# DanbiAubrey/Hypergraph_diffusion_for_recommendation

Hardware: AMD Instinct MI355X
Metric: hypergraph-conv fwd+bwd M-edges/sec at emb_dim=64; % HBM roofline (higher is better)
Workload: dtype f32

## Files before the change

hypergraph_diffusion_for_recommendation_amd/_native.py:

```python
from __future__ import annotations

import ctypes
import os
import threading

_HERE = os.path.dirname(os.path.abspath(__file__))
LIB_PATH = os.environ.get("HGD_LIB_PATH", os.path.join(_HERE, "_lib", "libhgd.so"))

c_void_p = ctypes.c_void_p
c_i64 = ctypes.c_int64
c_i32 = ctypes.c_int32
c_f32 = ctypes.c_float
c_f64 = ctypes.c_double
c_size = ctypes.c_size_t

HGD_OK = 0
EPI_NONE, EPI_LEAKY_RELU, EPI_RELU = 0, 1, 2
DT_F32, DT_BF16 = 0, 1
PACKED_IDX_BITS, PACKED_MAX_DICT = 22, 1024
ORDER_NONE, ORDER_MIN_COLUMN, ORDER_GREEDY = 0, 1, 2
ORDER_COL_CAP = 1024
_STATUS_NAMES = {0: "HGD_OK", 1: "HGD_ERR_INVALID_ARG", 2: "HGD_ERR_HIP",
                 3: "HGD_ERR_UNSUPPORTED", 4: "HGD_ERR_WORKSPACE"}

# ... 226 lines not shown
                                    c_i64, c_void_p, c_i32, c_i64, c_void_p, c_i32, c_i64, c_i32,
                                    c_i32, c_f32, c_i32, c_void_p, c_size, c_void_p]),
    "hgd_spmm_blocks_for_dt": (c_i32, [c_i64, c_i32, c_i32]),
    "hgd_spmm_row_order_for": (c_i32, [c_i64, c_i64, c_i64, c_i32]),
    "hgd_spmm_row_order_workspace_size": (c_size, [c_i64]),
    "hgd_spmm_row_order": (c_i32, [c_void_p, c_void_p, c_i64, c_i64, c_void_p, c_void_p,
                                   c_void_p, c_void_p, c_void_p, c_size, c_void_p]),
    "hgd_spmm_ordered": (c_i32, [c_void_p, c_void_p, c_void_p, c_void_p, c_i64, c_i64, c_i64,
                                 c_i64, c_void_p, c_i64, c_void_p, c_i64, c_i32, c_i32, c_f32,
                                 ctypes.POINTER(SplitPlan), c_void_p, c_size, c_void_p,
                                 c_void_p]),
    "hgd_spmm_block_order_for": (c_i32, [c_i64, c_i64, c_i64, c_i32, c_i32]),
    "hgd_spmm_col_blocks_ordered_workspace_size": (c_size, [c_i64, c_i32]),
    "hgd_spmm_col_blocks_ordered": (c_i32, [c_void_p, c_void_p, c_i64, c_i64, c_i32, c_void_p,
                                            c_void_p, c_void_p, c_void_p, c_void_p, c_size,
                                            c_void_p]),
    "hgd_spmm_blocked_ordered": (c_i32, [c_void_p, c_void_p, c_void_p, c_void_p, c_void_p, c_i64,
                                         c_i64, c_void_p, c_i64, c_void_p, c_i64, c_i32, c_i32,
                                         c_f32, c_i32, c_void_p]),
    "hgd_row_order_greedy": (c_i32, [c_void_p, c_void_p, c_i64, c_i64, c_i64, c_i32, c_i32, c_i32,
                                     c_i32, c_i32, c_void_p]),
    "hgd_col_block_order_greedy": (c_i32, [c_void_p, c_void_p, c_i64, c_i64, c_i32, c_i64, c_i32,
                                           c_i32, c_i32, c_i32, c_i32, c_void_p]),
    "hgd_spmm_row_order_from_workspace_size": (c_size, [c_i64]),
    "hgd_spmm_row_order_from": (c_i32, [c_void_p, c_void_p, c_void_p, c_i64, c_i64, c_void_p,
                                        c_void_p, c_void_p, c_void_p, c_size, c_void_p]),
    "hgd_spmm_col_blocks_ordered_from_workspace_size": (c_size, [c_i64, c_i32]),
    "hgd_spmm_col_blocks_ordered_from": (c_i32, [c_void_p, c_void_p, c_void_p, c_i64, c_i64, c_i32,
                                                 c_void_p, c_void_p, c_void_p, c_void_p, c_size,
                                                 c_void_p]),
    "hgd_spmm_order_geometry": (c_i32, [c_i32, c_i32, ctypes.POINTER(c_i32),
                                        ctypes.POINTER(c_i64)]),
    "hgd_spmm_row_order_kind_for": (c_i32, [c_i64, c_i64, c_i64, c_i32, c_i32]),
    "hgd_spmm_packed_for": (c_i32, [c_i64, c_i32, c_i64, c_i32]),
    "hgd_spmm_packed_fits": (c_i32, [c_i64, c_i32, c_i64, c_i32]),
    "hgd_spmm_pack_entries": (c_i32, [c_void_p, c_void_p, c_void_p, c_i64, c_i64, c_i64, c_i32,
                                      c_i32, c_i32, c_void_p, c_void_p]),
    "hgd_spmm_blocked_packed": (c_i32, [c_void_p, c_void_p, c_void_p, c_i32, c_i32, c_void_p,
                                        c_void_p, c_i64, c_i64, c_void_p, c_i64, c_void_p, c_i64,
                                        c_i32, c_i32, c_f32, c_i32, c_void_p]),
    "hgd_spmm_blocked_split_workspace_size": (c_size, [ctypes.POINTER(SplitPlan), c_i32, c_i32]),
    "hgd_spmm_blocked_split": (c_i32, [c_void_p, c_void_p, c_void_p, c_void_p, c_i64, c_i64,
                                       c_i64, c_i64, c_void_p, c_i64, c_void_p, c_i64, c_i32,
                                       c_i32, c_f32, c_i32, ctypes.POINTER(SplitPlan), c_void_p,
                                       c_size, c_void_p]),
    "hgd_spmm_blocks_split_for": (c_i32, [c_i64, c_i32, c_i64, c_i64, c_i32]),
# ... 381 lines not shown
```

hypergraph_diffusion_for_recommendation_amd/csrc/row_order_greedy.cpp:

```cpp
#include <algorithm>
#include <atomic>
#include <cstdarg>
#include <cstdint>
#include <cstdio>
#include <cstdlib>
#include <exception>
#include <new>
#include <thread>
#include <vector>

#include "../../include/hgd.h"

namespace hgd {

extern thread_local char g_last_error[512];

namespace {

hgd_status greedy_fail(hgd_status st, const char* fmt, ...) {
  va_list ap;
  va_start(ap, fmt);
  vsnprintf(g_last_error, sizeof(g_last_error), fmt, ap);
  va_end(ap);
  return st;
}

constexpr int kPickScan = 8;

struct Pieces {
  const int64_t* pb;
// ... 142 lines not shown
      const long v = std::strtol(e, nullptr, 10);
      if (v >= 1) t = v;
    }
  }
  t = std::min<int64_t>(t, n_tasks);
  return static_cast<int>(std::max<int64_t>(t, 1));
}

struct Task {
  Pieces p;
  const int32_t* rows;
  int64_t m;
  int32_t* out;
};

hgd_status run_tasks(const char* fn, const std::vector<Task>& tasks, int64_t window,
                     int64_t col_cap, int32_t threads) {
  std::atomic<size_t> next{0};
  std::atomic<int> bad_column{0}, no_memory{0};
  auto work = [&]() noexcept {
    for (size_t i = next.fetch_add(1); i < tasks.size(); i = next.fetch_add(1)) {
      const Task& t = tasks[i];
      try {
        if (!greedy_chunk(t.p, t.rows, t.m, window, col_cap, t.out)) bad_column.store(1);
      } catch (const std::exception&) {
        no_memory.store(1);
      }
    }
  };
  const int n = pick_threads(threads, static_cast<int64_t>(tasks.size()));
  std::vector<std::thread> th;
  try {
    th.reserve(static_cast<size_t>(n));
    for (int i = 1; i < n; ++i) th.emplace_back(work);
  } catch (const std::exception&) {
  }
  work();
  for (auto& t : th) t.join();
  if (bad_column.load())
    return greedy_fail(HGD_ERR_INVALID_ARG, "%s: a column outside [0, n_cols)", fn);
  if (no_memory.load()) return greedy_fail(HGD_ERR_WORKSPACE, "%s: out of host memory", fn);
  return HGD_OK;
}

void add_tasks(const Pieces& p, const int32_t* ne, int64_t m, int64_t R, int64_t X, int64_t C,
               int32_t* seq, std::vector<Task>& tasks, std::vector<int64_t>& part_off) {
  const int64_t n_wg = (m + R - 1) / R;
  part_off.assign(static_cast<size_t>(X) + 1, 0);
  for (int64_t x = 0; x < X; ++x) {
    const int64_t wgs = n_wg / X + (x < n_wg % X ? 1 : 0);
    int64_t size = wgs * R;
    if (n_wg > 0 && (n_wg - 1) % X == x) size -= n_wg * R - m;
    part_off[static_cast<size_t>(x) + 1] = part_off[static_cast<size_t>(x)] + size;
    for (int64_t c = 0; c < C; ++c) {
      const int64_t b = part_off[static_cast<size_t>(x)] + size * c / C;
      const int64_t e = part_off[static_cast<size_t>(x)] + size * (c + 1) / C;
      if (e > b) tasks.push_back(Task{p, ne + b, e - b, seq + b});
    }
  }
}

void place_parts(const int32_t* seq, const std::vector<int64_t>& part_off, int64_t R, int64_t X,
                 int32_t* order) {
  for (int64_t x = 0; x < X; ++x) {
    const int64_t off = part_off[static_cast<size_t>(x)];
    const int64_t size = part_off[static_cast<size_t>(x) + 1] - off;
    for (int64_t t = 0; t < size; ++t) order[(X * (t / R) + x) * R + t % R] = seq[off + t];
  }
}

hgd_status check_common(const char* fn, const int64_t* rowptr, const int32_t* col, int64_t n_rows,
                        int64_t n_cols, int64_t window, int32_t col_cap, int32_t rows_per_wg,
                        int32_t n_xcd, int32_t chunks_per_xcd, int32_t threads, const void* out) {
  if (n_rows < 0 || n_cols < 0) return greedy_fail(HGD_ERR_INVALID_ARG, "%s: negative sizes", fn);
  if (n_rows >= 0x7fffffffLL || n_cols >= 0x7fffffffLL)
    return greedy_fail(HGD_ERR_INVALID_ARG, "%s: n_rows / n_cols >= 2^31 - 1", fn);
  if (window < 1 || window > 0x7fffffffLL)
    return greedy_fail(HGD_ERR_INVALID_ARG, "%s: window must be 1..2^31-1 (got %lld)", fn,
                       static_cast<long long>(window));
  if (col_cap < 1) return greedy_fail(HGD_ERR_INVALID_ARG, "%s: col_cap must be >= 1", fn);
  if (rows_per_wg < 1 || n_xcd < 1 || chunks_per_xcd < 1)
    return greedy_fail(HGD_ERR_INVALID_ARG,
                       "%s: rows_per_wg, n_xcd and chunks_per_xcd must be >= 1", fn);
  if (threads < 0) return greedy_fail(HGD_ERR_INVALID_ARG, "%s: threads must be >= 0", fn);
  if (n_rows > 0 && (!rowptr || !out))
    return greedy_fail(HGD_ERR_INVALID_ARG, "%s: null rowptr / output", fn);
  if (n_rows > 0) {
    if (rowptr[0] < 0) return greedy_fail(HGD_ERR_INVALID_ARG, "%s: rowptr[0] < 0", fn);
    for (int64_t r = 0; r < n_rows; ++r)
      if (rowptr[r + 1] < rowptr[r])
        return greedy_fail(HGD_ERR_INVALID_ARG, "%s: rowptr descends at row %lld", fn,
                           static_cast<long long>(r));
    if (rowptr[n_rows] > rowptr[0] && !col)
      return greedy_fail(HGD_ERR_INVALID_ARG, "%s: null col", fn);
  }
  return HGD_OK;
}

}
}

extern "C" hgd_status hgd_row_order_greedy(const int64_t* rowptr, const int32_t* col,
                                           int64_t n_rows, int64_t n_cols, int64_t window,
                                           int32_t col_cap, int32_t rows_per_wg, int32_t n_xcd,
                                           int32_t chunks_per_xcd, int32_t threads,
                                           int32_t* order_out) {
  using namespace hgd;
  constexpr const char* fn = "hgd_row_order_greedy";
  g_last_error[0] = '\0';
  hgd_status s = check_common(fn, rowptr, col, n_rows, n_cols, window, col_cap, rows_per_wg, n_xcd,
                              chunks_per_xcd, threads, order_out);
  if (s != HGD_OK || n_rows == 0) return s;
  try {
    std::vector<int32_t> ne, seq;
    int64_t n_empty = 0;
    for (int64_t r = 0; r < n_rows; ++r)
      if (rowptr[r + 1] > rowptr[r]) ne.push_back(static_cast<int32_t>(r));
    const int64_t m = static_cast<int64_t>(ne.size());
    for (int64_t r = 0; r < n_rows; ++r)
      if (rowptr[r + 1] == rowptr[r]) order_out[m + n_empty++] = static_cast<int32_t>(r);
    seq.resize(ne.size());
    const Pieces p{rowptr, rowptr + 1, 1, col, 0, n_cols};
    std::vector<Task> tasks;
    std::vector<int64_t> part_off;
    add_tasks(p, ne.data(), m, rows_per_wg, n_xcd, chunks_per_xcd, seq.data(), tasks, part_off);
    s = run_tasks(fn, tasks, window, col_cap, threads);
    if (s != HGD_OK) return s;
    place_parts(seq.data(), part_off, rows_per_wg, n_xcd, order_out);
  } catch (const std::exception&) {
    return greedy_fail(HGD_ERR_WORKSPACE, "%s: out of host memory", fn);
  }
  return HGD_OK;
}

extern "C" hgd_status hgd_col_block_order_greedy(const int64_t* rowptr, const int32_t* col,
                                                 int64_t n_rows, int64_t n_cols, int32_t n_blocks,
                                                 int64_t window, int32_t col_cap,
                                                 int32_t rows_per_wg, int32_t n_xcd,
                                                 int32_t chunks_per_xcd, int32_t threads,
                                                 int32_t* blk_order_out) {
  using namespace hgd;
  constexpr const char* fn = "hgd_col_block_order_greedy";
  g_last_error[0] = '\0';
  if (n_blocks < 1 || n_blocks > 64)
    return greedy_fail(HGD_ERR_INVALID_ARG, "%s: blocks must be 1..64", fn);
  hgd_status s = check_common(fn, rowptr, col, n_rows, n_cols, window, col_cap, rows_per_wg, n_xcd,
                              chunks_per_xcd, threads, blk_order_out);
  if (s != HGD_OK || n_rows == 0) return s;
  try {
    const int64_t P = n_blocks;
    std::vector<int64_t> cut(static_cast<size_t>(n_rows) * static_cast<size_t>(P + 1));
    for (int64_t r = 0; r < n_rows; ++r) {
      int64_t* c = cut.data() + r * (P + 1);
      int64_t k = 0, prev = -1;
      c[0] = rowptr[r];
      for (int64_t j = rowptr[r]; j < rowptr[r + 1]; ++j) {
        const int64_t v = col[j];
        if (v < prev || v < 0 || v >= n_cols)
          return greedy_fail(HGD_ERR_INVALID_ARG,
                             "%s: row %lld's columns do not ascend inside [0, n_cols)", fn,
                             static_cast<long long>(r));
        prev = v;
        while (k + 1 < P && v >= n_cols * (k + 1) / P) c[++k] = j;
      }
      while (k < P) c[++k] = rowptr[r + 1];
    }
    std::vector<int32_t> ne(static_cast<size_t>(n_rows) * static_cast<size_t>(P));
    std::vector<int32_t> seq(ne.size());
    std::vector<int64_t> m(static_cast<size_t>(P), 0);
    std::vector<std::vector<int64_t>> part_off(static_cast<size_t>(P));
    std::vector<Task> tasks;
    for (int64_t k = 0; k < P; ++k) {
      int32_t* nek = ne.data() + k * n_rows;
      int32_t* outk = blk_order_out + k * n_rows;
      int64_t n_empty = 0, mk = 0;
      for (int64_t r = 0; r < n_rows; ++r)
        if (cut[r * (P + 1) + k + 1] > cut[r * (P + 1) + k]) nek[mk++] = static_cast<int32_t>(r);
      for (int64_t r = 0; r < n_rows; ++r)
        if (cut[r * (P + 1) + k + 1] == cut[r * (P + 1) + k])
          outk[mk + n_empty++] = static_cast<int32_t>(r);
      m[static_cast<size_t>(k)] = mk;
      const Pieces p{cut.data() + k, cut.data() + k + 1, P + 1, col, n_cols * k / P,
                     n_cols * (k + 1) / P};
      add_tasks(p, nek, mk, rows_per_wg, n_xcd, chunks_per_xcd, seq.data() + k * n_rows, tasks,
                part_off[static_cast<size_t>(k)]);
    }
    s = run_tasks(fn, tasks, window, col_cap, threads);
    if (s != HGD_OK) return s;
    for (int64_t k = 0; k < P; ++k)
      place_parts(seq.data() + k * n_rows, part_off[static_cast<size_t>(k)], rows_per_wg, n_xcd,
                  blk_order_out + k * n_rows);
  } catch (const std::exception&) {
    return greedy_fail(HGD_ERR_WORKSPACE, "%s: out of host memory", fn);
  }
  return HGD_OK;
}
```

hypergraph_diffusion_for_recommendation_amd/incidence.py:

```python
from __future__ import annotations

import copy
import ctypes
import os
import weakref
from typing import Dict, Optional, Tuple

import torch

from . import _native as nat
from . import profiling

DEFAULT_SPLIT_THRESHOLD = 2048
DEFAULT_SPLIT_CHUNK = 512
SPLIT_THRESHOLD_MIN = 128
SPLIT_NNZ_PER_THRESHOLD = 8192
SEGMENTED_MAX_AVG_DEGREE = 32
TARGET_GROUPS = 16384
ORDER_XCDS = 8
ORDER_CHUNKS_PER_XCD = 1


def auto_split(n_rows: int, nnz: int) -> Tuple[int, int]:
    if n_rows >= TARGET_GROUPS or nnz == 0:
        t = SPLIT_THRESHOLD_MIN
        while 2 * t <= nnz // SPLIT_NNZ_PER_THRESHOLD and t < DEFAULT_SPLIT_THRESHOLD:
            t *= 2
        return t, min(t // 2, DEFAULT_SPLIT_CHUNK)
    want = max(1, nnz // TARGET_GROUPS)
    chunk = 32
    while chunk < want and chunk < DEFAULT_SPLIT_CHUNK:
        chunk *= 2
    return 2 * chunk, chunk


def _ws(nbytes: int, device) -> torch.Tensor:
    return torch.empty(max(int(nbytes), 1), dtype=torch.uint8, device=device)


def _stream(device) -> int:
    return nat.stream_handle(device)


# ... 164 lines not shown
                ws = _ws(lib.hgd_split_plan_workspace_size(n), dev)
                for k, (n_heavy, n_chunks) in enumerate(counts.tolist()):
                    if n_heavy == 0:
                        continue
                    heavy_rows = torch.empty(n_heavy, dtype=torch.int32, device=dev)
                    heavy_cptr = torch.empty(n_heavy + 1, dtype=torch.int64, device=dev)
                    chunk_heavy = torch.empty(n_chunks, dtype=torch.int32, device=dev)
                    nat.check(lib.hgd_split_plan_build(
                        start.data_ptr() + 8 * k * n, n, thr, chunk, heavy_rows.data_ptr(),
                        heavy_cptr.data_ptr(), chunk_heavy.data_ptr(), n_heavy, n_chunks,
                        ws.data_ptr(), ws.numel(), st), "hgd_split_plan_build")
                    arrays.append((heavy_rows, heavy_cptr, chunk_heavy))
                    p = plans[k]
                    p.threshold, p.chunk = thr, chunk
                    p.n_heavy, p.n_chunks = n_heavy, n_chunks
                    p.heavy_rows = heavy_rows.data_ptr()
                    p.heavy_cptr = heavy_cptr.data_ptr()
                    p.chunk_heavy = chunk_heavy.data_ptr()
            got = self._col_block_plans[n_blocks] = (plans, arrays)
        return got[0]

    def _greedy_order(self, n_blocks: int, geom: tuple) -> torch.Tensor:
        window, rows_per_wg, n_xcd, chunks = geom
        rowptr, col = self.rowptr.cpu().contiguous(), self.col.cpu().contiguous()
        lib = nat.load()
        out = torch.empty(max(1, n_blocks) * self.n_rows, dtype=torch.int32)
        cp = col.data_ptr() if self.nnz else None
        if n_blocks:
            nat.check(lib.hgd_col_block_order_greedy(
                rowptr.data_ptr(), cp, self.n_rows, self.n_cols, n_blocks, window,
                nat.ORDER_COL_CAP, rows_per_wg, n_xcd, chunks, 0, out.data_ptr()),
                "hgd_col_block_order_greedy")
        else:
            nat.check(lib.hgd_row_order_greedy(
                rowptr.data_ptr(), cp, self.n_rows, self.n_cols, window, nat.ORDER_COL_CAP,
                rows_per_wg, n_xcd, chunks, 0, out.data_ptr()), "hgd_row_order_greedy")
        return out.to(self.device)

    def col_blocks_ordered(self, n_blocks: int, kind: int = nat.ORDER_MIN_COLUMN,
                           geom: Optional[tuple] = None) -> Tuple[torch.Tensor, ...]:
        if kind == nat.ORDER_GREEDY:
            return self._col_blocks_greedy(n_blocks, _need_geom(geom))
        got = self._col_blocks_ord.get(n_blocks)
        if got is None:
            if not self.cols_ascending:
                raise RuntimeError(
                    "col_blocks_ordered: the rows' columns are not known to be ascending")
            dev = self.device
            lib = nat.load()
            start = torch.empty(n_blocks * self.n_rows + 1, dtype=torch.int64, device=dev)
            bcol = torch.empty(self.nnz, dtype=torch.int32, device=dev)
            perm = torch.empty(self.nnz, dtype=torch.int32, device=dev)
            out_row = torch.empty(n_blocks * self.n_rows, dtype=torch.int32, device=dev)
            if self.n_rows:
                ws = _ws(lib.hgd_spmm_col_blocks_ordered_workspace_size(self.n_rows, n_blocks),
                         dev)
                nat.check(lib.hgd_spmm_col_blocks_ordered(
                    self.rowptr.data_ptr(), self.col.data_ptr() if self.nnz else None,
                    self.n_rows, self.n_cols, n_blocks, start.data_ptr(),
# ... 897 lines not shown
```

include/hgd.h:

```cpp
#ifndef HGD_H
#define HGD_H

#include <stddef.h>
#include <stdint.h>

#ifdef __cplusplus
extern "C" {
#endif

typedef enum hgd_status {
  HGD_OK = 0,
  HGD_ERR_INVALID_ARG = 1,
  HGD_ERR_HIP = 2,
  HGD_ERR_UNSUPPORTED = 3,
  HGD_ERR_WORKSPACE = 4
} hgd_status;

typedef enum hgd_epilogue {
  HGD_EPI_NONE = 0,
  HGD_EPI_LEAKY_RELU = 1,
  HGD_EPI_RELU = 2
} hgd_epilogue;

typedef enum hgd_tune_key {
// ... 109 lines not shown
                                       int64_t n_cols, int32_t n_blocks, int64_t* blk_start,
                                       int32_t* blk_col, int32_t* blk_perm, int32_t* blk_out_row,
                                       void* workspace, size_t workspace_bytes, void* stream);
hgd_status hgd_spmm_blocked_ordered(const int64_t* blk_start, const int32_t* blk_col,
                                    const float* blk_val, const float* blk_row_scale,
                                    const int32_t* blk_out_row, int64_t n_rows,
                                    int64_t n_src_rows, const float* X, int64_t ldx, float* Y,
                                    int64_t ldy, int32_t d, int32_t epilogue, float slope,
                                    int32_t n_blocks, void* stream);

#define HGD_ORDER_NONE 0
#define HGD_ORDER_MIN_COLUMN 1
#define HGD_ORDER_GREEDY 2
#define HGD_ORDER_COL_CAP 1024
hgd_status hgd_row_order_greedy(const int64_t* rowptr, const int32_t* col, int64_t n_rows,
                                int64_t n_cols, int64_t window, int32_t col_cap,
                                int32_t rows_per_wg, int32_t n_xcd, int32_t chunks_per_xcd,
                                int32_t threads, int32_t* order_out);
hgd_status hgd_col_block_order_greedy(const int64_t* rowptr, const int32_t* col, int64_t n_rows,
                                      int64_t n_cols, int32_t n_blocks, int64_t window,
                                      int32_t col_cap, int32_t rows_per_wg, int32_t n_xcd,
                                      int32_t chunks_per_xcd, int32_t threads,
                                      int32_t* blk_order_out);
size_t hgd_spmm_row_order_from_workspace_size(int64_t n_rows);
hgd_status hgd_spmm_row_order_from(const int32_t* order, const int64_t* rowptr, const int32_t* col,
                                   int64_t n_rows, int64_t n_cols, int64_t* rowptr_o,
                                   int32_t* col_o, int32_t* perm, void* workspace,
                                   size_t workspace_bytes, void* stream);
size_t hgd_spmm_col_blocks_ordered_from_workspace_size(int64_t n_rows, int32_t n_blocks);
hgd_status hgd_spmm_col_blocks_ordered_from(const int32_t* blk_order, const int64_t* rowptr,
                                            const int32_t* col, int64_t n_rows, int64_t n_cols,
                                            int32_t n_blocks, int64_t* blk_start, int32_t* blk_col,
                                            int32_t* blk_perm, void* workspace,
                                            size_t workspace_bytes, void* stream);
int32_t hgd_spmm_order_geometry(int32_t d, int32_t blocked, int32_t* rows_per_wg, int64_t* window);
int32_t hgd_spmm_row_order_kind_for(int64_t n_rows, int64_t n_src_rows, int64_t nnz, int32_t d,
                                    int32_t n_blocks);

#define HGD_SPMM_PACKED_MAX_DICT 1024
#define HGD_SPMM_PACKED_IDX_BITS 22
int32_t hgd_spmm_packed_fits(int64_t n_src_rows, int32_t n_blocks, int64_t n_dict,
                             int32_t idx_bits);
int32_t hgd_spmm_packed_for(int64_t n_src_rows, int32_t n_blocks, int64_t n_dict,
                            int32_t idx_bits);
hgd_status hgd_spmm_pack_entries(const int64_t* blk_start, const int32_t* blk_col,
                                 const int32_t* src_code, int64_t n_rows, int64_t n_src_rows,
// ... 608 lines not shown
```

Before: 7393.

## Add pooled multi-XCD greedy row ordering with a parallel team walk

Result: faster. 7641 (median of 6 runs) (+3.4%).

```diff
diff --git a/hypergraph_diffusion_for_recommendation_amd/_native.py b/hypergraph_diffusion_for_recommendation_amd/_native.py
--- a/hypergraph_diffusion_for_recommendation_amd/_native.py
+++ b/hypergraph_diffusion_for_recommendation_amd/_native.py
@@ -272,6 +272,10 @@
                                      c_i32, c_i32, c_void_p]),
     "hgd_col_block_order_greedy": (c_i32, [c_void_p, c_void_p, c_i64, c_i64, c_i32, c_i64, c_i32,
                                            c_i32, c_i32, c_i32, c_i32, c_void_p]),
+    "hgd_row_order_greedy_pooled": (c_i32, [c_void_p, c_void_p, c_i64, c_i64, c_i64, c_i32, c_i32,
+                                            c_i32, c_i32, c_i32, c_void_p]),
+    "hgd_col_block_order_greedy_pooled": (c_i32, [c_void_p, c_void_p, c_i64, c_i64, c_i32, c_i64,
+                                                  c_i32, c_i32, c_i32, c_i32, c_i32, c_void_p]),
     "hgd_spmm_row_order_from_workspace_size": (c_size, [c_i64]),
     "hgd_spmm_row_order_from": (c_i32, [c_void_p, c_void_p, c_void_p, c_i64, c_i64, c_void_p,
                                         c_void_p, c_void_p, c_void_p, c_size, c_void_p]),
diff --git a/hypergraph_diffusion_for_recommendation_amd/csrc/row_order_greedy.cpp b/hypergraph_diffusion_for_recommendation_amd/csrc/row_order_greedy.cpp
--- a/hypergraph_diffusion_for_recommendation_amd/csrc/row_order_greedy.cpp
+++ b/hypergraph_diffusion_for_recommendation_amd/csrc/row_order_greedy.cpp
@@ -5,7 +5,10 @@
 #include <cstdio>
 #include <cstdlib>
 #include <exception>
+#include <limits>
+#include <memory>
 #include <new>
+#include <stdexcept>
 #include <thread>
 #include <vector>
 
@@ -194,51 +197,600 @@
     for (size_t i = next.fetch_add(1); i < tasks.size(); i = next.fetch_add(1)) {
       const Task& t = tasks[i];
       try {
-        if (!greedy_chunk(t.p, t.rows, t.m, window, col_cap, t.out)) bad_column.store(1);
+          if (!greedy_chunk(t.p, t.rows, t.m, window, col_cap, t.out)) bad_column.store(1);
+        } catch (const std::exception&) {
+          no_memory.store(1);
+        }
+      }
+    };
+    const int n = pick_threads(threads, static_cast<int64_t>(tasks.size()));
+    std::vector<std::thread> th;
+    try {
+      th.reserve(static_cast<size_t>(n));
+      for (int i = 1; i < n; ++i) th.emplace_back(work);
+    } catch (const std::exception&) {
+    }
+    work();
+    for (auto& t : th) t.join();
+    if (bad_column.load())
+      return greedy_fail(HGD_ERR_INVALID_ARG, "%s: a column outside [0, n_cols)", fn);
+    if (no_memory.load()) return greedy_fail(HGD_ERR_WORKSPACE, "%s: out of host memory", fn);
+    return HGD_OK;
+  }
+
+  void add_tasks(const Pieces& p, const int32_t* ne, int64_t m, int64_t R, int64_t X, int64_t C,
+                 int32_t* seq, std::vector<Task>& tasks, std::vector<int64_t>& part_off) {
+    const int64_t n_wg = (m + R - 1) / R;
+    part_off.assign(static_cast<size_t>(X) + 1, 0);
+    for (int64_t x = 0; x < X; ++x) {
+      const int64_t wgs = n_wg / X + (x < n_wg % X ? 1 : 0);
+      int64_t size = wgs * R;
+      if (n_wg > 0 && (n_wg - 1) % X == x) size -= n_wg * R - m;
+      part_off[static_cast<size_t>(x) + 1] = part_off[static_cast<size_t>(x)] + size;
+      for (int64_t c = 0; c < C; ++c) {
+        const int64_t b = part_off[static_cast<size_t>(x)] + size * c / C;
+        const int64_t e = part_off[static_cast<size_t>(x)] + size * (c + 1) / C;
+        if (e > b) tasks.push_back(Task{p, ne + b, e - b, seq + b});
+      }
+    }
+  }
+
+  void place_parts(const int32_t* seq, const std::vector<int64_t>& part_off, int64_t R, int64_t X,
+                   int32_t* order) {
+    for (int64_t x = 0; x < X; ++x) {
+      const int64_t off = part_off[static_cast<size_t>(x)];
+      const int64_t size = part_off[static_cast<size_t>(x) + 1] - off;
+      for (int64_t t = 0; t < size; ++t) order[(X * (t / R) + x) * R + t % R] = seq[off + t];
+    }
+  }
+
+  constexpr int kMaxOwners = 16;
+  constexpr int64_t kMaxRowsPerRound = 8, kRoundShare = 128;
+
+  class TeamBarrier {
+   public:
+    explicit TeamBarrier(int n) : n_(n) {}
+    void wait() {
+      if (n_ == 1) return;
+      const int g = gen_.load(std::memory_order_acquire);
+      if (count_.fetch_add(1, std::memory_order_acq_rel) + 1 == n_) {
+        count_.store(0, std::memory_order_relaxed);
+        gen_.store(g + 1, std::memory_order_release);
+        return;
+      }
+      for (int spin = 0; gen_.load(std::memory_order_acquire) == g; ++spin)
+        if (spin >= 512) std::this_thread::yield();
+    }
+
+   private:
+    const int n_;
+    std::atomic<int> count_{0}, gen_{0};
+  };
+
+  struct Pool {
+    Pieces p;
+    const int32_t* rows;
+    int64_t m;
+    int32_t* seq;
+    std::vector<int64_t> size, off;
+    int64_t nnz, max_len;
+    int K;
+  };
+
+  struct alignas(64) Proposal {
+    int32_t cnt, n;
+    int32_t row[kPickScan];
+    uint16_t len[kPickScan];
+  };
+  static_assert(sizeof(Proposal) == 64, "a proposal is a cache line");
+
+  constexpr int kRecentCols = 32;
+  constexpr int kStackLook = 64;
+
+  template <class Cnt>
+  struct Owner {
+    static constexpr Cnt kPlaced = std::numeric_limits<Cnt>::max();
+    int64_t lo = 0, n = 0;
+    std::vector<uint32_t> tptr;
+    std::vector<int32_t> tl, len;
+    std::vector<Cnt> cnt;
+    std::vector<std::vector<int32_t>> stack;
+    std::vector<int32_t> top;
+    std::vector<uint8_t> mark;
+    int64_t live = 0, gone = 0;
+  };
+
+  template <class Cnt>
+  struct PoolState {
+    std::vector<Owner<Cnt>> owners;
+    std::vector<int32_t> key, by_min, coldeg;
+    std::vector<uint8_t> placed;
+    std::vector<int32_t> in_fifo;
+    std::vector<std::vector<int32_t>> fifo;
+    std::vector<int64_t> fifo_at, fifo_n;
+    std::vector<std::vector<uint32_t>> events;
+    std::vector<int32_t> recent;
+    std::vector<int64_t> recent_n;
+    std::vector<Proposal> prop;
+    std::atomic<int> bad_column{0}, no_memory{0};
+    std::atomic<int> fail_apply{0}, fail_fifo{0};
+  };
+
+  struct Team {
+    explicit Team(int n) : size(n), barrier(n) {}
+    int size;
+    TeamBarrier barrier;
+    void* state = nullptr;
+  };
+
+  template <class Cnt>
+  bool build_owner(const Pool& pl, int G, Owner<Cnt>& o, int32_t* key) {
+    const Pieces& p = pl.p;
+    const int64_t nc = p.c_hi - p.c_lo;
+    o.tptr.assign(static_cast<size_t>(nc) + 1, 0);
+    o.len.resize(static_cast<size_t>(o.n));
+    uint64_t total = 0;
+    for (int64_t i = 0; i < o.n; ++i) {
+      const int32_t r = pl.rows[o.lo + i];
+      const int64_t b = p.begin(r), e = p.end(r);
+      int64_t lo = nc;
+      for (int64_t j = b; j < e; ++j) {
+        const int64_t c = static_cast<int64_t>(p.col[j]) - p.c_lo;
+        if (c < 0 || c >= nc) return false;
+        ++o.tptr[static_cast<size_t>(c) + 1];
+        lo = std::min(lo, c);
+      }
+      key[o.lo + i] = static_cast<int32_t>(lo);
+      o.len[static_cast<size_t>(i)] = static_cast<int32_t>(e - b);
+      total += static_cast<uint64_t>(e - b);
+    }
+    if (total > 0xffffffffull) throw std::length_error("an owner's lists");
+    for (size_t c = 0; c < static_cast<size_t>(nc); ++c) o.tptr[c + 1] += o.tptr[c];
+    o.tl.resize(static_cast<size_t>(total));
+    {
+      std::vector<uint32_t> fill(o.tptr.begin(), o.tptr.end() - 1);
+      for (int64_t i = 0; i < o.n; ++i) {
+        const int32_t r = pl.rows[o.lo + i];
+        for (int64_t j = p.begin(r), e = p.end(r); j < e; ++j)
+          o.tl[fill[static_cast<size_t>(p.col[j] - p.c_lo)]++] = static_cast<int32_t>(i);
+      }
+    }
+    o.cnt.assign(static_cast<size_t>(G) * static_cast<size_t>(o.n), 0);
+    o.stack.assign(static_cast<size_t>(G) * static_cast<size_t>(pl.max_len + 1), {});
+    o.top.assign(static_cast<size_t>(G), 0);
+    o.mark.assign(static_cast<size_t>(o.n), 0);
+    o.live = o.n;
+    return true;
+  }
+
+  template <class Cnt>
+  void pack_lists(Owner<Cnt>& o) {
+    const size_t nc = o.tptr.size() - 1;
+    uint32_t w = 0, j = 0;
+    for (size_t c = 0; c < nc; ++c) {
+      const uint32_t e = o.tptr[c + 1];
+      o.tptr[c] = w;
+      for (; j < e; ++j)
+        if (o.cnt[static_cast<size_t>(o.tl[j])] != Owner<Cnt>::kPlaced) o.tl[w++] = o.tl[j];
+    }
+    o.tptr[nc] = w;
+    o.live -= o.gone;
+    o.gone = 0;
+  }
+
+  inline void offer(Proposal& out, int32_t len32, int32_t row) {
+    const uint16_t len = static_cast<uint16_t>(std::min<int32_t>(len32, 0xffff));
+    for (int i = 0; i < out.n; ++i)
+      if (out.row[i] == row) return;
+    int at = out.n++;
+    for (; at > 0 && (out.len[at - 1] > len || (out.len[at - 1] == len && out.row[at - 1] > row));
+         --at) {
+      out.len[at] = out.len[at - 1];
+      out.row[at] = out.row[at - 1];
+    }
+    out.len[at] = len;
+    out.row[at] = row;
+  }
+
+  template <class Cnt>
+  void sweep(Owner<Cnt>& o, const Cnt* cn, std::vector<int32_t>& st, int32_t b) {
+    size_t w = st.size();
+    for (size_t i = st.size(); i-- > 0;) {
+      const int32_t t = st[i];
+      if (static_cast<int32_t>(cn[t]) != b || o.mark[static_cast<size_t>(t)]) continue;
+      o.mark[static_cast<size_t>(t)] = 1;
+      st[--w] = t;
+    }
+    for (size_t i = w; i < st.size(); ++i) o.mark[static_cast<size_t>(st[i])] = 0;
+    st.erase(st.begin(), st.begin() + static_cast<std::ptrdiff_t>(w));
+  }
+
+  template <class Cnt>
+  void propose(Owner<Cnt>& o, int g, int64_t max_len, const int32_t* recent, int64_t recent_n,
+               Proposal& out) {
+    const Cnt* const cn = o.cnt.data() + static_cast<size_t>(g) * static_cast<size_t>(o.n);
+    std::vector<int32_t>* const stk =
+        o.stack.data() + static_cast<size_t>(g) * static_cast<size_t>(max_len + 1);
+    int32_t top = o.top[static_cast<size_t>(g)];
+    for (; top >= 2; --top) {
+      std::vector<int32_t>& st = stk[top];
+      while (!st.empty() && static_cast<int32_t>(cn[st.back()]) != top) st.pop_back();
+      if (!st.empty()) break;
+    }
+    o.top[static_cast<size_t>(g)] = top;
+    out.n = 0;
+    if (top >= 2) {
+      out.cnt = top;
+      const std::vector<int32_t>& st = stk[top];
+      const size_t stop = st.size() > kStackLook ? st.size() - kStackLook : 0;
+      for (size_t i = st.size(); i-- > stop && out.n < kPickScan;) {
+        const int32_t t = st[i];
+        if (static_cast<int32_t>(cn[t]) == top)
+          offer(out, o.len[static_cast<size_t>(t)], static_cast<int32_t>(o.lo + t));
+      }
+      return;
+    }
+    out.cnt = 1;
+    const int64_t back = std::min<int64_t>(recent_n, kRecentCols);
+    for (int64_t q = 1; q <= back && out.n < kPickScan; ++q) {
+      const size_t c = static_cast<size_t>(recent[(recent_n - q) % kRecentCols]);
+      for (uint32_t j = o.tptr[c], e = o.tptr[c + 1]; j < e && out.n < kPickScan; ++j) {
+        const int32_t t = o.tl[j];
+        if (cn[t] != Owner<Cnt>::kPlaced && cn[t] >= 1)
+          offer(out, o.len[static_cast<size_t>(t)], static_cast<int32_t>(o.lo + t));
+      }
+    }
+  }
+
+  template <class Cnt>
+  void apply_round(Owner<Cnt>& o, int G, int64_t max_len,
+                   const std::vector<std::vector<uint32_t>>& events, std::vector<uint64_t>& evs,
+                   std::vector<uint64_t>& moves) {
+    constexpr size_t kAhead = 8, kMoveAhead = 16;
+    evs.clear();
+    moves.clear();
+    for (int g = 0; g < G; ++g)
+      for (const uint32_t ev : events[static_cast<size_t>(g)])
+        evs.push_back(static_cast<uint64_t>(ev) << 16 | static_cast<uint64_t>(g));
+    const uint32_t* const tptr = o.tptr.data();
+    const int32_t* const tl = o.tl.data();
+    const size_t ne = evs.size();
+    for (size_t i = 0; i < std::min(ne, 2 * kAhead); ++i) __builtin_prefetch(tptr + (evs[i] >> 17));
+    for (size_t i = 0; i < std::min(ne, kAhead); ++i) __builtin_prefetch(tl + tptr[evs[i] >> 17]);
+    for (size_t i = 0; i < ne; ++i) {
+      if (i + 2 * kAhead < ne) __builtin_prefetch(tptr + (evs[i + 2 * kAhead] >> 17));
+      if (i + kAhead < ne) __builtin_prefetch(tl + tptr[evs[i + kAhead] >> 17]);
+      const size_t c = static_cast<size_t>(evs[i] >> 17);
+      const uint64_t low = (evs[i] & 0xffffu) << 1 | (evs[i] >> 16 & 1u);
+      for (uint32_t j = tptr[c], e = tptr[c + 1]; j < e; ++j)
+        moves.push_back(static_cast<uint64_t>(static_cast<uint32_t>(tl[j])) << 32 | low);
+    }
+    Cnt* const cnt = o.cnt.data();
+    const size_t n = static_cast<size_t>(o.n), nm = moves.size();
+    const size_t sweep_at = 2 * n + 256;
+    auto at = [&](uint64_t mv) { return cnt + (mv >> 1 & 0xffffu) * n + (mv >> 32); };
+    for (size_t i = 0; i < std::min(nm, kMoveAhead); ++i) __builtin_prefetch(at(moves[i]), 1);
+    for (size_t i = 0; i < nm; ++i) {
+      if (i + kMoveAhead < nm) __builtin_prefetch(at(moves[i + kMoveAhead]), 1);
+      const uint64_t mv = moves[i];
+      Cnt* const cn = at(mv);
+      const Cnt b = *cn;
+      if (b == Owner<Cnt>::kPlaced) continue;
+      int32_t to;
+      if (mv & 1u) {
+        *cn = static_cast<Cnt>(b + 1);
+        if (b < 1) continue;
+        to = static_cast<int32_t>(b) + 1;
+      } else {
+        if (b < 1) continue;
+        *cn = static_cast<Cnt>(b - 1);
+        if (b < 3) continue;
+        to = static_cast<int32_t>(b) - 1;
+      }
+      const size_t g = mv >> 1 & 0xffffu;
+      std::vector<int32_t>& st =
+          o.stack[g * static_cast<size_t>(max_len + 1) + static_cast<size_t>(to)];
+      if (st.size() >= sweep_at) sweep(o, cnt + g * n, st, to);
+      st.push_back(static_cast<int32_t>(mv >> 32));
+      if ((mv & 1u) && to > o.top[g]) o.top[g] = to;
+    }
+  }
+
+  template <class Cnt>
+  int walk_pool(Team& team, int me, const Pool& pl, int64_t window, int64_t col_cap) {
+    const int G = static_cast<int>(pl.size.size());
+    const int K = pl.K, T = team.size;
+    const Pieces& p = pl.p;
+    const int64_t nc = p.c_hi - p.c_lo, m = pl.m;
+    const int k_lo = K * me / T, k_hi = K * (me + 1) / T;
+    window = std::min<int64_t>(window, std::max<int64_t>(1, pl.nnz));
+
+    if (me == 0) {
+      PoolState<Cnt>* made = nullptr;
+      try {
+        made = new PoolState<Cnt>();
+        made->owners.resize(static_cast<size_t>(K));
+        for (int k = 0; k < K; ++k) {
+          made->owners[static_cast<size_t>(k)].lo = m * k / K;
+          made->owners[static_cast<size_t>(k)].n = m * (k + 1) / K - m * k / K;
+        }
+        made->key.resize(static_cast<size_t>(m));
+        made->by_min.resize(static_cast<size_t>(m));
+        made->coldeg.assign(static_cast<size_t>(nc), 0);
+        made->placed.assign(static_cast<size_t>(m), 0);
+        made->in_fifo.assign(static_cast<size_t>(G) * static_cast<size_t>(nc), 0);
+        made->fifo.resize(static_cast<size_t>(G));
+        for (int g = 0; g < G; ++g)
+          made->fifo[static_cast<size_t>(g)].resize(
+              static_cast<size_t>(std::min(window, pl.size[static_cast<size_t>(g)] * pl.max_len)));
+        made->fifo_at.assign(static_cast<size_t>(G), 0);
+        made->fifo_n.assign(static_cast<size_t>(G), 0);
+        made->events.resize(static_cast<size_t>(G));
+        made->recent.assign(static_cast<size_t>(G) * kRecentCols, 0);
+        made->recent_n.assign(static_cast<size_t>(G), 0);
+        made->prop.resize(static_cast<size_t>(K) * static_cast<size_t>(G));
       } catch (const std::exception&) {
-        no_memory.store(1);
-      }
-    }
-  };
-  const int n = pick_threads(threads, static_cast<int64_t>(tasks.size()));
+        delete made;
+        made = nullptr;
+      }
+      team.state = made;
+    }
+    team.barrier.wait();
+    PoolState<Cnt>* const st = static_cast<PoolState<Cnt>*>(team.state);
+    if (!st) {
+      team.barrier.wait();
+      return 2;
+    }
+
+    for (int k = k_lo; k < k_hi; ++k) {
+      try {
+        if (!build_owner(pl, G, st->owners[static_cast<size_t>(k)], st->key.data()))
+          st->bad_column.store(1);
+      } catch (const std::exception&) {
+        st->no_memory.store(1);
+      }
+    }
+    team.barrier.wait();
+    int bad = st->bad_column.load() ? 1 : st->no_memory.load() ? 2 : 0;
+    if (!bad) {
+      for (int64_t c = nc * me / T, e = nc * (me + 1) / T; c < e; ++c) {
+        int64_t deg = 0;
+        for (int k = 0; k < K; ++k) {
+          const Owner<Cnt>& o = st->owners[static_cast<size_t>(k)];
+          deg += o.tptr[static_cast<size_t>(c) + 1] - o.tptr[static_cast<size_t>(c)];
+        }
+        st->coldeg[static_cast<size_t>(c)] =
+            static_cast<int32_t>(std::min<int64_t>(deg, 0x7fffffff));
+      }
+      if (me == T - 1) {
+      try {
+          std::vector<int64_t> at(static_cast<size_t>(nc) + 2, 0);
+          const int32_t* const key = st->key.data();
+          for (int64_t i = 0; i < m; ++i) ++at[static_cast<size_t>(key[i]) + 1];
+          for (size_t c = 0; c <= static_cast<size_t>(nc); ++c) at[c + 1] += at[c];
+          for (int64_t i = 0; i < m; ++i)
+            st->by_min[static_cast<size_t>(at[static_cast<size_t>(key[i])]++)] =
+                static_cast<int32_t>(i);
+      } catch (const std::exception&) {
+        st->no_memory.store(1);
+      }
+    }
+    team.barrier.wait();
+    bad = st->no_memory.load() ? 2 : 0;
+  }
+
+  if (!bad) {
+    const int64_t B = std::clamp<int64_t>(window * m / (kRoundShare * pl.nnz), 1, kMaxRowsPerRound);
+    int64_t longest = 0;
+    for (int g = 0; g < G; ++g) longest = std::max(longest, pl.size[static_cast<size_t>(g)]);
+    int64_t fall = 0;
+    std::vector<int32_t> pick;
+    std::vector<uint64_t> evs, moves;
+    try {
+      pick.resize(static_cast<size_t>(G) * static_cast<size_t>(B));
+    } catch (const std::exception&) {
+      st->fail_apply.store(1);
+    }
+    const uint8_t* const placed = st->placed.data();
+    const int32_t* const by_min = st->by_min.data();
+    for (int64_t s0 = 0; s0 < longest; s0 += B) {
+      for (int k = k_lo; k < k_hi; ++k)
+        for (int g = 0; g < G; ++g)
+          if (s0 < pl.size[static_cast<size_t>(g)])
+            propose(st->owners[static_cast<size_t>(k)], g, pl.max_len,
+                    st->recent.data() + static_cast<size_t>(g) * kRecentCols,
+                    st->recent_n[static_cast<size_t>(g)],
+                    st->prop[static_cast<size_t>(g) * static_cast<size_t>(K) +
+                             static_cast<size_t>(k)]);
+      team.barrier.wait();
+      if (st->fail_apply.load()) break;
+      for (size_t i = 0; i < st->prop.size(); ++i) __builtin_prefetch(&st->prop[i]);
+      size_t n_pick = 0;
+      auto taken = [&](int32_t row) {
+        for (size_t h = 0; h < n_pick; ++h)
+          if (pick[h] == row) return true;
+        return false;
+      };
+      for (int64_t s = s0; s < s0 + B; ++s)
+        for (int g = 0; g < G; ++g, ++n_pick) {
+          pick[n_pick] = -1;
+          if (s >= pl.size[static_cast<size_t>(g)]) continue;
+          int32_t best = -1, best_cnt = 0, best_len = 0;
+          for (int k = 0; k < K; ++k) {
+            const Proposal& pr = st->prop[static_cast<size_t>(g) * static_cast<size_t>(K) +
+                                          static_cast<size_t>(k)];
+            if (pr.n == 0 || (best >= 0 && pr.cnt < best_cnt)) continue;
+            for (int i = 0; i < pr.n; ++i) {
+              if (taken(pr.row[i])) continue;
+              if (best < 0 || pr.cnt > best_cnt || pr.len[i] < best_len) {
+                best = pr.row[i];
+                best_cnt = pr.cnt;
+                best_len = pr.len[i];
+              }
+              break;
+            }
+          }
+          if (best < 0) {
+            while (placed[by_min[fall]] || taken(by_min[fall])) ++fall;
+            best = by_min[fall];
+          }
+          pick[n_pick] = best;
+        }
+      try {
+        for (int g = me; g < G; g += T) {
+          std::vector<uint32_t>& ev = st->events[static_cast<size_t>(g)];
+          ev.clear();
+          int32_t* const fifo = st->fifo[static_cast<size_t>(g)].data();
+          const int64_t cap = static_cast<int64_t>(st->fifo[static_cast<size_t>(g)].size());
+          int32_t* const in_fifo =
+              st->in_fifo.data() + static_cast<size_t>(g) * static_cast<size_t>(nc);
+          int64_t& fifo_at = st->fifo_at[static_cast<size_t>(g)];
+          int64_t& fifo_n = st->fifo_n[static_cast<size_t>(g)];
+          int32_t* const recent = st->recent.data() + static_cast<size_t>(g) * kRecentCols;
+          int64_t& recent_n = st->recent_n[static_cast<size_t>(g)];
+          for (int64_t i = 0; i < B; ++i) {
+            const int32_t at = pick[static_cast<size_t>(i) * static_cast<size_t>(G) +
+                                    static_cast<size_t>(g)];
+            if (at < 0) continue;
+            const int32_t r = pl.rows[at];
+            pl.seq[pl.off[static_cast<size_t>(g)] + s0 + i] = r;
+            for (int64_t j = p.begin(r), e = p.end(r); j < e; ++j) {
+              const int64_t c = static_cast<int64_t>(p.col[j]) - p.c_lo;
+              int64_t slot;
+              if (fifo_n == cap) {
+                const int64_t o = fifo[fifo_at];
+                if (--in_fifo[o] == 0 && st->coldeg[static_cast<size_t>(o)] <= col_cap)
+                  ev.push_back(static_cast<uint32_t>(o) << 1);
+                slot = fifo_at;
+                fifo_at = fifo_at + 1 == cap ? 0 : fifo_at + 1;
+              } else {
+                slot = fifo_at + fifo_n;
+                if (slot >= cap) slot -= cap;
+                ++fifo_n;
+              }
+              fifo[slot] = static_cast<int32_t>(c);
+              if (in_fifo[c]++ == 0 && st->coldeg[static_cast<size_t>(c)] <= col_cap) {
+                ev.push_back((static_cast<uint32_t>(c) << 1) | 1u);
+                recent[recent_n++ % kRecentCols] = static_cast<int32_t>(c);
+              }
+            }
+          }
+        }
+      } catch (const std::exception&) {
+        st->fail_fifo.store(1);
+      }
+      team.barrier.wait();
+      if (st->fail_fifo.load()) break;
+      try {
+        for (int k = k_lo; k < k_hi; ++k) {
+          Owner<Cnt>& o = st->owners[static_cast<size_t>(k)];
+          for (size_t h = 0; h < n_pick; ++h) {
+            const int64_t t = static_cast<int64_t>(pick[h]) - o.lo;
+            if (pick[h] < 0 || t < 0 || t >= o.n) continue;
+            for (int g = 0; g < G; ++g)
+              o.cnt[static_cast<size_t>(g) * static_cast<size_t>(o.n) + static_cast<size_t>(t)] =
+                  Owner<Cnt>::kPlaced;
+            st->placed[static_cast<size_t>(o.lo + t)] = 1;
+            ++o.gone;
+          }
+          if (o.gone >= 64 && o.gone * 4 >= o.live) pack_lists(o);
+          apply_round(o, G, pl.max_len, st->events, evs, moves);
+        }
+      } catch (const std::exception&) {
+        st->fail_apply.store(1);
+      }
+    }
+  }
+  team.barrier.wait();
+  if (st->fail_apply.load() || st->fail_fifo.load()) bad = 2;
+  team.barrier.wait();
+  if (me == 0) {
+    delete st;
+    team.state = nullptr;
+  }
+  return bad;
+}
+
+int walk_pool_any(Team& team, int me, const Pool& pl, int64_t window, int64_t col_cap) {
+  if (pl.max_len < 0xff) return walk_pool<uint8_t>(team, me, pl, window, col_cap);
+  if (pl.max_len < 0xffff) return walk_pool<uint16_t>(team, me, pl, window, col_cap);
+  return walk_pool<int32_t>(team, me, pl, window, col_cap);
+}
+
+void add_pools(const Pieces& p, const int32_t* ne, int64_t m, int64_t R, int64_t X, int64_t G,
+               int32_t* seq, std::vector<Pool>& pools, std::vector<int64_t>& part_off) {
+  std::vector<Task> unused;
+  add_tasks(p, ne, m, R, X, 1, seq, unused, part_off);
+  for (int64_t q = 0; q < X / G; ++q) {
+    const int64_t b = part_off[static_cast<size_t>(q * G)];
+    const int64_t e = part_off[static_cast<size_t>((q + 1) * G)];
+    if (e == b) continue;
+    Pool pl{p, ne + b, e - b, seq + b, {}, {}, 0, 0, 1};
+    for (int64_t g = 0; g < G; ++g) {
+      pl.off.push_back(part_off[static_cast<size_t>(q * G + g)] - b);
+      pl.size.push_back(part_off[static_cast<size_t>(q * G + g) + 1] -
+                        part_off[static_cast<size_t>(q * G + g)]);
+    }
+    for (int64_t i = b; i < e; ++i) {
+      const int64_t len = p.end(ne[i]) - p.begin(ne[i]);
+      pl.nnz += len;
+      pl.max_len = std::max(pl.max_len, len);
+    }
+    const int64_t deg = pl.nnz / std::max<int64_t>(1, p.c_hi - p.c_lo);
+    while (pl.K * 2 <= kMaxOwners && pl.K * 4 <= deg) pl.K *= 2;
+    pools.push_back(std::move(pl));
+  }
+}
+
+hgd_status run_pools(const char* fn, const std::vector<Pool>& pools, int64_t window,
+                     int64_t col_cap, int32_t threads) {
+  if (pools.empty()) return HGD_OK;
+  int64_t owners = 0;
+  for (const Pool& pl : pools) owners += pl.K;
+  std::atomic<int> bad_column{0}, no_memory{0};
+  std::atomic<int> go{0};
+  std::vector<std::unique_ptr<Team>> teams;
+  auto work = [&](int id) noexcept {
+    int n;
+    for (int spin = 0; (n = go.load(std::memory_order_acquire)) == 0; ++spin)
+      if (spin >= 512) std::this_thread::yield();
+    if (n < 0) return;
+    const int n_teams = static_cast<int>(teams.size());
+    Team& team = *teams[static_cast<size_t>(id % n_teams)];
+    for (size_t i = static_cast<size_t>(id % n_teams); i < pools.size();
+         i += static_cast<size_t>(n_teams)) {
+      const int bad = walk_pool_any(team, id / n_teams, pools[i], window, col_cap);
+      if (bad == 1) bad_column.store(1);
+      if (bad == 2) no_memory.store(1);
+    }
+  };
+  int n = 1;
   std::vector<std::thread> th;
   try {
-    th.reserve(static_cast<size_t>(n));
-    for (int i = 1; i < n; ++i) th.emplace_back(work);
+    const int want = pick_threads(threads, owners);
+    th.reserve(static_cast<size_t>(want));
+    for (int i = 1; i < want; ++i) {
+      th.emplace_back(work, i);
+      ++n;
+    }
   } catch (const std::exception&) {
   }
-  work();
+  try {
+    const int n_teams = static_cast<int>(std::min<size_t>(pools.size(), static_cast<size_t>(n)));
+    for (int i = 0; i < n_teams; ++i)
+      teams.emplace_back(new Team(n / n_teams + (i < n % n_teams ? 1 : 0)));
+  } catch (const std::exception&) {
+    go.store(-1, std::memory_order_release);
+    for (auto& t : th) t.join();
+    return greedy_fail(HGD_ERR_WORKSPACE, "%s: out of host memory", fn);
+  }
+  go.store(n, std::memory_order_release);
+  work(0);
   for (auto& t : th) t.join();
   if (bad_column.load())
     return greedy_fail(HGD_ERR_INVALID_ARG, "%s: a column outside [0, n_cols)", fn);
   if (no_memory.load()) return greedy_fail(HGD_ERR_WORKSPACE, "%s: out of host memory", fn);
   return HGD_OK;
-}
-
-void add_tasks(const Pieces& p, const int32_t* ne, int64_t m, int64_t R, int64_t X, int64_t C,
-               int32_t* seq, std::vector<Task>& tasks, std::vector<int64_t>& part_off) {
-  const int64_t n_wg = (m + R - 1) / R;
-  part_off.assign(static_cast<size_t>(X) + 1, 0);
-  for (int64_t x = 0; x < X; ++x) {
-    const int64_t wgs = n_wg / X + (x < n_wg % X ? 1 : 0);
-    int64_t size = wgs * R;
-    if (n_wg > 0 && (n_wg - 1) % X == x) size -= n_wg * R - m;
-    part_off[static_cast<size_t>(x) + 1] = part_off[static_cast<size_t>(x)] + size;
-    for (int64_t c = 0; c < C; ++c) {
-      const int64_t b = part_off[static_cast<size_t>(x)] + size * c / C;
-      const int64_t e = part_off[static_cast<size_t>(x)] + size * (c + 1) / C;
-      if (e > b) tasks.push_back(Task{p, ne + b, e - b, seq + b});
-    }
-  }
-}
-
-void place_parts(const int32_t* seq, const std::vector<int64_t>& part_off, int64_t R, int64_t X,
-                 int32_t* order) {
-  for (int64_t x = 0; x < X; ++x) {
-    const int64_t off = part_off[static_cast<size_t>(x)];
-    const int64_t size = part_off[static_cast<size_t>(x) + 1] - off;
-    for (int64_t t = 0; t < size; ++t) order[(X * (t / R) + x) * R + t % R] = seq[off + t];
-  }
 }
 
 hgd_status check_common(const char* fn, const int64_t* rowptr, const int32_t* col, int64_t n_rows,
@@ -269,16 +821,10 @@
   return HGD_OK;
 }
 
-}
-}
-
-extern "C" hgd_status hgd_row_order_greedy(const int64_t* rowptr, const int32_t* col,
-                                           int64_t n_rows, int64_t n_cols, int64_t window,
-                                           int32_t col_cap, int32_t rows_per_wg, int32_t n_xcd,
-                                           int32_t chunks_per_xcd, int32_t threads,
-                                           int32_t* order_out) {
-  using namespace hgd;
-  constexpr const char* fn = "hgd_row_order_greedy";
+hgd_status row_order(const char* fn, const int64_t* rowptr, const int32_t* col, int64_t n_rows,
+                     int64_t n_cols, int64_t window, int32_t col_cap, int32_t rows_per_wg,
+                     int32_t n_xcd, int32_t chunks_per_xcd, int32_t xcds_per_pool, int32_t threads,
+                     int32_t* order_out) {
   g_last_error[0] = '\0';
   hgd_status s = check_common(fn, rowptr, col, n_rows, n_cols, window, col_cap, rows_per_wg, n_xcd,
                               chunks_per_xcd, threads, order_out);
@@ -295,8 +841,14 @@
     const Pieces p{rowptr, rowptr + 1, 1, col, 0, n_cols};
     std::vector<Task> tasks;
     std::vector<int64_t> part_off;
-    add_tasks(p, ne.data(), m, rows_per_wg, n_xcd, chunks_per_xcd, seq.data(), tasks, part_off);
-    s = run_tasks(fn, tasks, window, col_cap, threads);
+    if (xcds_per_pool > 1) {
+      std::vector<Pool> pools;
+      add_pools(p, ne.data(), m, rows_per_wg, n_xcd, xcds_per_pool, seq.data(), pools, part_off);
+      s = run_pools(fn, pools, window, col_cap, threads);
+    } else {
+      add_tasks(p, ne.data(), m, rows_per_wg, n_xcd, chunks_per_xcd, seq.data(), tasks, part_off);
+      s = run_tasks(fn, tasks, window, col_cap, threads);
+    }
     if (s != HGD_OK) return s;
     place_parts(seq.data(), part_off, rows_per_wg, n_xcd, order_out);
   } catch (const std::exception&) {
@@ -305,14 +857,10 @@
   return HGD_OK;
 }
 
-extern "C" hgd_status hgd_col_block_order_greedy(const int64_t* rowptr, const int32_t* col,
-                                                 int64_t n_rows, int64_t n_cols, int32_t n_blocks,
-                                                 int64_t window, int32_t col_cap,
-                                                 int32_t rows_per_wg, int32_t n_xcd,
-                                                 int32_t chunks_per_xcd, int32_t threads,
-                                                 int32_t* blk_order_out) {
-  using namespace hgd;
-  constexpr const char* fn = "hgd_col_block_order_greedy";
+hgd_status block_order(const char* fn, const int64_t* rowptr, const int32_t* col, int64_t n_rows,
+                       int64_t n_cols, int32_t n_blocks, int64_t window, int32_t col_cap,
+                       int32_t rows_per_wg, int32_t n_xcd, int32_t chunks_per_xcd,
+                       int32_t xcds_per_pool, int32_t threads, int32_t* blk_order_out) {
   g_last_error[0] = '\0';
   if (n_blocks < 1 || n_blocks > 64)
     return greedy_fail(HGD_ERR_INVALID_ARG, "%s: blocks must be 1..64", fn);
@@ -342,6 +890,7 @@
     std::vector<int64_t> m(static_cast<size_t>(P), 0);
     std::vector<std::vector<int64_t>> part_off(static_cast<size_t>(P));
     std::vector<Task> tasks;
+    std::vector<Pool> pools;
     for (int64_t k = 0; k < P; ++k) {
       int32_t* nek = ne.data() + k * n_rows;
       int32_t* outk = blk_order_out + k * n_rows;
@@ -354,10 +903,15 @@
       m[static_cast<size_t>(k)] = mk;
       const Pieces p{cut.data() + k, cut.data() + k + 1, P + 1, col, n_cols * k / P,
                      n_cols * (k + 1) / P};
-      add_tasks(p, nek, mk, rows_per_wg, n_xcd, chunks_per_xcd, seq.data() + k * n_rows, tasks,
-                part_off[static_cast<size_t>(k)]);
-    }
-    s = run_tasks(fn, tasks, window, col_cap, threads);
+      if (xcds_per_pool > 1)
+        add_pools(p, nek, mk, rows_per_wg, n_xcd, xcds_per_pool, seq.data() + k * n_rows, pools,
+                  part_off[static_cast<size_t>(k)]);
+      else
+        add_tasks(p, nek, mk, rows_per_wg, n_xcd, chunks_per_xcd, seq.data() + k * n_rows, tasks,
+                  part_off[static_cast<size_t>(k)]);
+    }
+    s = xcds_per_pool > 1 ? run_pools(fn, pools, window, col_cap, threads)
+                          : run_tasks(fn, tasks, window, col_cap, threads);
     if (s != HGD_OK) return s;
     for (int64_t k = 0; k < P; ++k)
       place_parts(seq.data() + k * n_rows, part_off[static_cast<size_t>(k)], rows_per_wg, n_xcd,
@@ -367,3 +921,59 @@
   }
   return HGD_OK;
 }
+
+hgd_status check_pool(const char* fn, int32_t n_xcd, int32_t xcds_per_pool) {
+  if (xcds_per_pool < 1 || n_xcd < 1 || n_xcd % xcds_per_pool != 0)
+    return greedy_fail(HGD_ERR_INVALID_ARG,
+                       "%s: n_xcd and xcds_per_pool must be >= 1, and the second divide the first",
+                       fn);
+  if (xcds_per_pool > 64)
+    return greedy_fail(HGD_ERR_INVALID_ARG, "%s: xcds_per_pool must be <= 64", fn);
+  return HGD_OK;
+}
+
+}
+}
+
+extern "C" hgd_status hgd_row_order_greedy(const int64_t* rowptr, const int32_t* col,
+                                           int64_t n_rows, int64_t n_cols, int64_t window,
+                                           int32_t col_cap, int32_t rows_per_wg, int32_t n_xcd,
+                                           int32_t chunks_per_xcd, int32_t threads,
+                                           int32_t* order_out) {
+  return hgd::row_order("hgd_row_order_greedy", rowptr, col, n_rows, n_cols, window, col_cap,
+                        rows_per_wg, n_xcd, chunks_per_xcd, 0, threads, order_out);
+}
+
+extern "C" hgd_status hgd_col_block_order_greedy(const int64_t* rowptr, const int32_t* col,
+                                                 int64_t n_rows, int64_t n_cols, int32_t n_blocks,
+                                                 int64_t window, int32_t col_cap,
+                                                 int32_t rows_per_wg, int32_t n_xcd,
+                                                 int32_t chunks_per_xcd, int32_t threads,
+                                                 int32_t* blk_order_out) {
+  return hgd::block_order("hgd_col_block_order_greedy", rowptr, col, n_rows, n_cols, n_blocks,
+                          window, col_cap, rows_per_wg, n_xcd, chunks_per_xcd, 0, threads,
+                          blk_order_out);
+}
+
+extern "C" hgd_status hgd_row_order_greedy_pooled(const int64_t* rowptr, const int32_t* col,
+                                                  int64_t n_rows, int64_t n_cols, int64_t window,
+                                                  int32_t col_cap, int32_t rows_per_wg,
+                                                  int32_t n_xcd, int32_t xcds_per_pool,
+                                                  int32_t threads, int32_t* order_out) {
+  constexpr const char* fn = "hgd_row_order_greedy_pooled";
+  hgd::g_last_error[0] = '\0';
+  if (hgd::check_pool(fn, n_xcd, xcds_per_pool) != HGD_OK) return HGD_ERR_INVALID_ARG;
+  return hgd::row_order(fn, rowptr, col, n_rows, n_cols, window, col_cap, rows_per_wg, n_xcd, 1,
+                        xcds_per_pool, threads, order_out);
+}
+
+extern "C" hgd_status hgd_col_block_order_greedy_pooled(
+    const int64_t* rowptr, const int32_t* col, int64_t n_rows, int64_t n_cols, int32_t n_blocks,
+    int64_t window, int32_t col_cap, int32_t rows_per_wg, int32_t n_xcd, int32_t xcds_per_pool,
+    int32_t threads, int32_t* blk_order_out) {
+  constexpr const char* fn = "hgd_col_block_order_greedy_pooled";
+  hgd::g_last_error[0] = '\0';
+  if (hgd::check_pool(fn, n_xcd, xcds_per_pool) != HGD_OK) return HGD_ERR_INVALID_ARG;
+  return hgd::block_order(fn, rowptr, col, n_rows, n_cols, n_blocks, window, col_cap, rows_per_wg,
+                          n_xcd, 1, xcds_per_pool, threads, blk_order_out);
+}
diff --git a/hypergraph_diffusion_for_recommendation_amd/incidence.py b/hypergraph_diffusion_for_recommendation_amd/incidence.py
--- a/hypergraph_diffusion_for_recommendation_amd/incidence.py
+++ b/hypergraph_diffusion_for_recommendation_amd/incidence.py
@@ -19,6 +19,16 @@
 TARGET_GROUPS = 16384
 ORDER_XCDS = 8
 ORDER_CHUNKS_PER_XCD = 1
+ORDER_XCDS_PER_POOL = 8
+
+
+def order_pool_width() -> int:
+    env = os.environ.get("HGD_SPMM_ORDER_POOL", "")
+    if env == "":
+        return ORDER_XCDS_PER_POOL
+    if env not in ("1", "2", "4", "8"):
+        raise ValueError(f"HGD_SPMM_ORDER_POOL must be 1, 2, 4 or 8, got {env!r}")
+    return int(env)
 
 
 def auto_split(n_rows: int, nnz: int) -> Tuple[int, int]:
@@ -229,19 +239,22 @@
 
     def _greedy_order(self, n_blocks: int, geom: tuple) -> torch.Tensor:
         window, rows_per_wg, n_xcd, chunks = geom
+        pool = order_pool_width() if n_xcd > 1 else 0
+        if pool == 1 and chunks != 1:
+            pool = 0
+        if pool and n_xcd % pool:
+            raise ValueError(f"a pool of {pool} XCDs does not divide the geometry's {n_xcd}")
         rowptr, col = self.rowptr.cpu().contiguous(), self.col.cpu().contiguous()
         lib = nat.load()
         out = torch.empty(max(1, n_blocks) * self.n_rows, dtype=torch.int32)
         cp = col.data_ptr() if self.nnz else None
-        if n_blocks:
-            nat.check(lib.hgd_col_block_order_greedy(
-                rowptr.data_ptr(), cp, self.n_rows, self.n_cols, n_blocks, window,
-                nat.ORDER_COL_CAP, rows_per_wg, n_xcd, chunks, 0, out.data_ptr()),
-                "hgd_col_block_order_greedy")
-        else:
-            nat.check(lib.hgd_row_order_greedy(
-                rowptr.data_ptr(), cp, self.n_rows, self.n_cols, window, nat.ORDER_COL_CAP,
-                rows_per_wg, n_xcd, chunks, 0, out.data_ptr()), "hgd_row_order_greedy")
+        name = ("hgd_col_block_order_greedy" if n_blocks else "hgd_row_order_greedy") + \
+            ("_pooled" if pool else "")
+        args = (rowptr.data_ptr(), cp, self.n_rows, self.n_cols) + \
+            ((n_blocks,) if n_blocks else ()) + \
+            (window, nat.ORDER_COL_CAP, rows_per_wg, n_xcd, pool if pool else chunks, 0,
+             out.data_ptr())
+        nat.check(getattr(lib, name)(*args), name)
         return out.to(self.device)
 
     def col_blocks_ordered(self, n_blocks: int, kind: int = nat.ORDER_MIN_COLUMN,
diff --git a/include/hgd.h b/include/hgd.h
--- a/include/hgd.h
+++ b/include/hgd.h
@@ -155,6 +155,15 @@
                                       int32_t col_cap, int32_t rows_per_wg, int32_t n_xcd,
                                       int32_t chunks_per_xcd, int32_t threads,
                                       int32_t* blk_order_out);
+hgd_status hgd_row_order_greedy_pooled(const int64_t* rowptr, const int32_t* col, int64_t n_rows,
+                                       int64_t n_cols, int64_t window, int32_t col_cap,
+                                       int32_t rows_per_wg, int32_t n_xcd, int32_t xcds_per_pool,
+                                       int32_t threads, int32_t* order_out);
+hgd_status hgd_col_block_order_greedy_pooled(const int64_t* rowptr, const int32_t* col,
+                                             int64_t n_rows, int64_t n_cols, int32_t n_blocks,
+                                             int64_t window, int32_t col_cap, int32_t rows_per_wg,
+                                             int32_t n_xcd, int32_t xcds_per_pool,
+                                             int32_t threads, int32_t* blk_order_out);
 size_t hgd_spmm_row_order_from_workspace_size(int64_t n_rows);
 hgd_status hgd_spmm_row_order_from(const int32_t* order, const int64_t* rowptr, const int32_t* col,
                                    int64_t n_rows, int64_t n_cols, int64_t* rowptr_o,
```
